# google/guetzli

Hardware: AMD Instinct MI355X
Metric: MPix/s encoded at --quality 95 (higher is better)
Workload: dtype f32+f64 (butteraugli), int32/int16 (DCT/quantize/entropy coding); 1 GPU; single 3840x2160 sRGB image, --quality 95 (BASELINE configs[2]), whole guetzli::Process per step (host RGB in, JPEG bytes out), 1 image per GPU per step; 12 timed steps after 5 warm-up between barrier + synchronise, max over ranks; images_per_gpu=1, steps=12, warmup=5, output_bytes=2895866

## Files before the change

guetzli_amd/csrc/api/chain.h:

```cpp
#pragma once

namespace {
static bool packed_blur(const gz_ctx* c) {
  if (c->cfg.blur_packed >= 0) return c->cfg.blur_packed != 0;
  return (size_t)c->w * c->h >= 1500000;
}
constexpr int kTileRows = 32;
constexpr int kSmallTileRows = 16;
static bool small_tiles(const gz_ctx* c) {
  if (c->cfg.tile_rows == 16) return true;
  if (c->cfg.tile_rows == 32) return false;
  return (size_t)c->w * c->h < 7000000;
}

template <int R, class Src, int NC, bool PAIR = false>
int blur_h(gz_ctx* c, hipStream_t stream, const SrcPack<Src, NC>& src, const PlanePack<NC>& dst,
           const BlurCfg& cfg, const BlurCfg* second = nullptr) {
  if (PAIR != (second != nullptr)) { c->err = "blur pair mismatch"; return GZ_E_STATE; }
  const BlurCfg& cfg1 = PAIR ? *second : cfg;
  if (cfg.r != R || cfg1.r != R) { c->err = "blur radius mismatch"; return GZ_E_STATE; }
  const Taps<R> t0 = taps_of<R>(cfg), t1 = taps_of<R>(cfg1);
  const BorderScale b0 = cfg.bx, b1 = cfg1.bx;
  const int w = c->w, h = c->h, pitch = c->pitch;
  if (packed_blur(c)) {
// ... 77 lines not shown
  make_taps_host(sigma, cfg);
  cfg->border_ratio = border_ratio;
  std::vector<float> xl, xh, yl, yh;
  border_scales_host(*cfg, c->w, &xl, &xh);
  border_scales_host(*cfg, c->h, &yl, &yh);
  const int r = cfg->r;
  if (ctx_owns) TRY(regrow(c, nullptr, nullptr, 0, {{(void**)&cfg->d_scale, sizeof(float) * 4 * r}}));
  else HIPCHK(c, pool_malloc((void**)&cfg->d_scale, sizeof(float) * 4 * r));
  std::vector<float> all;
  all.insert(all.end(), xl.begin(), xl.end());
  all.insert(all.end(), xh.begin(), xh.end());
  all.insert(all.end(), yl.begin(), yl.end());
  all.insert(all.end(), yh.begin(), yh.end());
  HIPCHK(c, hipMemcpy(cfg->d_scale, all.data(), sizeof(float) * 4 * r, hipMemcpyHostToDevice));
  cfg->bx.lo = cfg->d_scale;
  cfg->bx.hi = cfg->d_scale + r;
  cfg->by.lo = cfg->d_scale + 2 * r;
  cfg->by.hi = cfg->d_scale + 3 * r;
  return GZ_OK;
}

static bool single_stream_wanted(const gz_ctx* c) {
  if (c->cfg.single_stream >= 0) return c->cfg.single_stream != 0;
  return slots_taken(c->device) > 1;
}
struct ChainStreams {
  hipStream_t main, side, side2;
};
static ChainStreams chain_streams(const gz_ctx* c, bool forked) {
  return forked ? ChainStreams{c->stream, c->side_stream, c->side_stream2} : ChainStreams{c->stream, c->stream, c->stream};
}
static int record_for(gz_ctx* c, hipStream_t from, hipStream_t to, hipEvent_t ev) {
  if (from != to) HIPCHK(c, hipEventRecord(ev, from));
  return GZ_OK;
}
static int wait_for(gz_ctx* c, hipStream_t from, hipStream_t to, hipEvent_t ev) {
  if (from != to) HIPCHK(c, hipStreamWaitEvent(to, ev, 0));
  return GZ_OK;
}
static int fork(gz_ctx* c, hipStream_t from, hipStream_t to, hipEvent_t ev) {
  TRY(record_for(c, from, to, ev));
  return wait_for(c, from, to, ev);
}

int stage_opsin(gz_ctx* c, hipStream_t stream, const int* tiles = nullptr, int n_tiles = 0) {
  SrcPack<SrcPlain, 3> s;
  for (int i = 0; i < 3; ++i) s.s[i].p = c->lin[i];
  PostOpsin post;
  for (int i = 0; i < 3; ++i) { post.lin[i] = c->lin[i]; post.xyb[i] = c->xyb[i]; }
  return blur2d<2, 3, SrcPlain, PostOpsin>(c, stream, s, post, c->blur[B_OPSIN], BlockMaxOut{nullptr, nullptr, 0, tiles}, n_tiles);
}
static int opsin_tile_rows(const gz_ctx*) { return kSmallTileRows; }

int stage_separate(gz_ctx* c, const ChainStreams& cs, Psycho* ps) {
  c->have_map_plane = false;
  TRY(fork(c, cs.main, cs.side2, c->ev_xyb));
  {
    SrcPack<SrcPlain, 1> s; PlanePack<1> t;
    s.s[0].p = c->xyb[2]; t.p[0] = c->distmap;
    TRY((blur_h<16, SrcPlain, 1>(c, cs.side2, s, t, c->blur[B_LF])));
  }
  {
    SrcPack<SrcPlain, 2> s; PlanePack<2> t; CPlanePack<2> ct;
    for (int i = 0; i < 2; ++i) { s.s[i].p = c->xyb[i]; t.p[i] = c->tmp[i]; ct.p[i] = c->tmp[i]; }
    TRY((blur_h<16, SrcPlain, 2>(c, cs.main, s, t, c->blur[B_LF])));
    PostLFxy post;
    for (int i = 0; i < 2; ++i) { post.lf_raw[i] = c->lf_raw[i]; post.lf_vals[i] = ps->lfv[i]; }
    TRY((blur_v<16, 2, PostLFxy>(c, cs.main, ct, post, c->blur[B_LF])));
  }
  TRY(fork(c, cs.main, cs.side2, c->ev_lfy));
  {
    CPlanePack<1> ct; ct.p[0] = c->distmap;
    PostLFb post; post.lf_raw_y = c->lf_raw[1]; post.lf_vals_b = ps->lfv[2];
    TRY((blur_v<16, 1, PostLFb>(c, cs.side2, ct, post, c->blur[B_LF])));
  }
  {
    SrcPack<SrcDiff, 2> s;
    for (int i = 0; i < 2; ++i) {
      s.s[i].a = c->xyb[i];
      s.s[i].b = c->lf_raw[i];
    }
    PostMF post;
    for (int i = 0; i < 2; ++i) {
      post.xyb[i] = c->xyb[i];
      post.lf_raw[i] = c->lf_raw[i];
      post.mf[i] = ps->mf[i];
      post.hf_pre[i] = c->hfp[i];
    }
    TRY((blur2d<8, 2, SrcDiff, PostMF>(c, cs.main, s, post, c->blur[B_MF])));
  }
  {
    SrcPack<SrcPlain, 2> s;
    for (int i = 0; i < 2; ++i) s.s[i].p = c->hfp[i];
    PostHF post;
    for (int i = 0; i < 2; ++i) {
      post.hf_pre[i] = c->hfp[i];
      post.hf[i] = ps->hf[i];
      post.uhf[i] = ps->uhf[i];
    }
    post.lf_raw_y = c->lf_raw[1];
    TRY((blur2d<4, 2, SrcPlain, PostHF>(c, cs.main, s, post, c->blur[B_HF])));
  }
  return GZ_OK;
}

int stage_mask_blurs(gz_ctx* c, hipStream_t stream, hipStream_t small_stream, const MaskPrePack& pk) {
  dim3 grid(gz_div_up(c->w, 1024), c->h, 2);
  GZ_LAUNCH(k_mask_pre, grid, dim3(256), stream, pk, c->w, c->h, c->pitch);
  KCHK(c);
  TRY(fork(c, stream, small_stream, c->ev_mask_pre));
  {
    SrcPack<SrcPlain, 2> s; PlanePack<2> t; CPlanePack<2> ct;
    s.s[0].p = c->diffx; s.s[1].p = c->diffy;
    t.p[0] = c->tmp[1]; t.p[1] = c->tmp[2];
    ct.p[0] = c->tmp[1]; ct.p[1] = c->tmp[2];
    TRY((blur_h<20, SrcPlain, 2, true>(c, stream, s, t, c->blur[B_MASKX], &c->blur[B_MASKY1])));
    PostStore<2> post; post.out[0] = c->mxb; post.out[1] = c->myb2;
    TRY((blur_v<20, 2, PostStore<2>, true>(c, stream, ct, post, c->blur[B_MASKX], &c->blur[B_MASKY1])));
  }
  {
    SrcPack<SrcPlain, 1> s; s.s[0].p = c->diffy;
// ... 338 lines not shown
```

guetzli_amd/csrc/api/entry_probes.h:

```cpp
#pragma once

extern "C" {

#ifndef GZ_NO_PROBES

int gz_probe_blur(gz_ctx* c, const float* in, float sigma, float border_ratio, float* out) {
  DeviceScope ds_(c);
  if (!c || !in || !out) return GZ_E_ARG;
  BlurCfg cfg;
  int rc = setup_blur_cfg(c, &cfg, sigma, border_ratio, false);
  float* src = c->xyb[0];
  c->xyb_is_cand = false;
  if (rc == GZ_OK) rc = upload_planes(c, in, &src, 1);
  SrcPack<SrcPlain, 1> s; s.s[0].p = src;
  PostStore<1> post; post.out[0] = c->xyb[1];
  if (rc == GZ_OK) rc = blur_plane(c, c->stream, s, c->tmp[0], post, cfg);
  if (rc == GZ_OK) rc = download_plane(c, c->xyb[1], out);
  (void)hipStreamSynchronize(c->stream);
  (void)pool_free(cfg.d_scale);
  return rc;
}

int gz_probe_opsin(gz_ctx* c, const float* rgb3, float* xyb3) {
  DeviceScope ds_(c);
  if (!c || !rgb3 || !xyb3) return GZ_E_ARG;
  c->lin_is_cand = c->xyb_is_cand = false;
  TRY(upload_planes(c, rgb3, c->lin, 3));
  TRY(stage_opsin(c, c->stream));
  for (int i = 0; i < 3; ++i) TRY(download_plane(c, c->xyb[i], xyb3 + (size_t)i * c->w * c->h));
  HIPCHK(c, hipStreamSynchronize(c->stream));
  return GZ_OK;
}

int gz_probe_separate_frequencies(gz_ctx* c, const float* xyb3, float* out10) {
  DeviceScope ds_(c);
  if (!c || !xyb3 || !out10) return GZ_E_ARG;
  TRY(ensure_pip(c));
  c->xyb_is_cand = false;
  TRY(upload_planes(c, xyb3, c->xyb, 3));
  TRY(stage_separate(c, chain_streams(c, false), &c->pip));
  const size_t n = (size_t)c->w * c->h;
  for (int i = 0; i < 3; ++i) TRY(download_plane(c, c->pip.lfv[i], out10 + i * n));
  for (int i = 0; i < 2; ++i) TRY(download_plane(c, c->pip.mf[i], out10 + (3 + i) * n));
  memset(out10 + 5 * n, 0, sizeof(float) * n);
  for (int i = 0; i < 2; ++i) TRY(download_plane(c, c->pip.hf[i], out10 + (6 + i) * n));
  for (int i = 0; i < 2; ++i) TRY(download_plane(c, c->pip.uhf[i], out10 + (8 + i) * n));
  HIPCHK(c, hipStreamSynchronize(c->stream));
  return GZ_OK;
}

int gz_probe_diffmap(gz_ctx* c, const float* rgb0, const float* rgb1, float* diffmap,
                     float* score) {
  DeviceScope ds_(c);
  if (!c || !rgb0 || !rgb1) return GZ_E_ARG;
  TRY(ensure_pip(c));
  c->lin_is_cand = c->xyb_is_cand = false;
  TRY(upload_planes(c, rgb0, c->lin, 3));
  TRY(stage_opsin(c, c->stream));
  TRY(stage_separate(c, chain_streams(c, false), &c->pip));
  TRY(upload_planes(c, rgb1, c->lin, 3));
  TRY(stage_opsin(c, c->stream));
  TRY(stage_separate(c, chain_streams(c, false), &c->pi1));
  TRY(stage_diffmap(c, chain_streams(c, !single_stream_wanted(c)), c->pip, c->pi1, kWantDistmap, ClearMax::kMemset));
  if (diffmap) TRY(download_plane(c, c->distmap, diffmap));
  unsigned bits = 0;
  HIPCHK(c, hipMemcpyAsync(&bits, c->d_max_bits, 4, hipMemcpyDeviceToHost, c->stream));
  HIPCHK(c, hipStreamSynchronize(c->stream));
  if (score) memcpy(score, &bits, 4);
  return GZ_OK;
}

int gz_probe_mask(gz_ctx* c, const float* xyb0, const float* xyb1, float* mask3,
                  float* mask_dc3) {
  DeviceScope ds_(c);
  if (!c || !xyb0 || !xyb1 || !mask3) return GZ_E_ARG;
  TRY(ensure_pip(c));
  float* a[2] = {c->pip.hf[0], c->pip.hf[1]};
  float* b[2] = {c->pi1.hf[0], c->pi1.hf[1]};
  TRY(upload_planes(c, xyb0, a, 2));
  TRY(upload_planes(c, xyb1, b, 2));
  const float* const ca2[2] = {a[0], a[1]};
  const float* const cb2[2] = {b[0], b[1]};
  MaskPrePack pk;
  TRY(mask_pack_plain(c, c->stream, ca2, cb2, &pk));
  TRY(stage_mask_blurs(c, c->stream, c->stream, pk));
  TRY(launch_combine(c, c->stream, combine_mask_args(c, c->mask_out, c->mask_dc_out)));
  const size_t n = (size_t)c->w * c->h;
  for (int i = 0; i < 3; ++i) {
    TRY(download_plane(c, c->mask_out[i], mask3 + i * n));
    if (mask_dc3) TRY(download_plane(c, c->mask_dc_out[i], mask_dc3 + i * n));
  }
  HIPCHK(c, hipStreamSynchronize(c->stream));
  return GZ_OK;
// ... 308 lines not shown
```

guetzli_amd/csrc/gz_kernels_blur.h:

```cpp
#pragma once
#include "gz_common.h"
#include "gz_math.h"

namespace gz {

template <int R>
struct Taps {
  float k[2 * R + 1];
  float ks[2 * R + 1];
};

struct BorderScale {
  const float* lo;
  const float* hi;
};

struct SrcPlain {
  const float* p;
  GZ_DEVFN float operator()(size_t idx) const { return GZ_LDG(p, idx); }
  GZ_DEVFN gz_f4 load4(size_t idx) const { return GZ_LDG4(p, idx); }
};
struct SrcDiff {
  const float* a;
  const float* b;
// ... 490 lines not shown
    if (c > 0) __syncthreads();
    for (int ry = tg; ry < TH + 2 * R; ry += 4) {
      const int y = y0 - R + ry;
      float v = 0.0f;
      if (x < w && y >= 0 && y < h) v = in[(size_t)y * pitch + x];
      tile[ry][tx] = v;
    }
    __syncthreads();
#pragma unroll 1
    for (int i = 0; i < VPTt; ++i) {
      const int ly = tg * VPTt + i;
      const int y = y0 + ly;
      float sum = 0.0f;
      if (y < h) {
        const bool border = y < R || y >= h - R;
        const float* col = &tile[ly][tx];
        if (!border) {
#pragma unroll
          for (int j = 0; j <= 2 * R; ++j) sum += col[j * VW] * taps.ks[j];
        } else {
#pragma unroll
          for (int j = 0; j <= 2 * R; ++j) sum += col[j * VW] * taps.k[j];
          sum = sum * (y < R ? bs.lo[y] : bs.hi[h - 1 - y]);
        }
      }
      if constexpr (ZCH) {
        float* __restrict__ o = bid.z == 1 ? post.out[1] : post.out[0];
        if (x < w && y < h) o[(size_t)y * pitch + x] = sum;
      } else if (NC > 1) {
        outv[c][ly][tx] = sum;
      } else {
        float v1[1] = {sum};
        if (x < w && y < h) (void)post((size_t)y * pitch + x, v1);
      }
    }
  }
  if constexpr (NCL > 1) {
#pragma unroll 1
    for (int i = 0; i < VPTt; ++i) {
      const int ly = tg * VPTt + i;
      const int y = y0 + ly;
      if (x < w && y < h) {
        float v[NC];
#pragma unroll
        for (int c = 0; c < NC; ++c) v[c] = outv[c][ly][tx];
        (void)post((size_t)y * pitch + x, v);
      }
    }
  }
}

constexpr int T2 = 64;

template <int R, int NC, class Src, class Post, bool BM, int TH>
__global__ __launch_bounds__(256, 4) void k_blur2d(SrcPack<Src, NC> src, Post post, int w, int h,
                                                int pitch, Taps<R> taps, BorderScale bsx,
                                                BorderScale bsy, BlockMaxOut bm) {
  constexpr bool ROLL = !BM;
  constexpr int RA = (R + 3) & ~3;
  constexpr int IW = T2 + 2 * RA;
  constexpr int IH = TH + 2 * R;
  constexpr int VPTt = TH / 4;
  constexpr int OFF = RA - R;
  __shared__ __attribute__((aligned(16))) float tile[IH][IW];
  const int tid = threadIdx.x;
  GzTile bid;
  if (bm.tiles) {
    const int t = bm.tiles[blockIdx.x], gx = (w + T2 - 1) / T2;
    bid.x = t % gx; bid.y = t / gx; bid.z = 0;
  } else {
    bid = gz_xcd_tile();
  }
  const int x0 = bid.x * T2, y0 = bid.y * TH;
  const bool interior = x0 >= RA && x0 + T2 + RA <= w && y0 >= R && y0 + TH + R <= h &&
                        (pitch & 3) == 0;
  const int tx = tid & 63, tg = tid >> 6;
  constexpr int kRowSlotShift = (IW / 4) & 15;
  const int hr = tid >> 4;
  const int hq = (((tid & 15) - (hr & 1) * kRowSlotShift) & 15) * 4;
  float acc[ROLL ? 1 : NC][VPTt];
  __shared__ __attribute__((aligned(16))) float outv[ROLL ? NC : 1][ROLL ? TH : 1][T2];
  constexpr int kChannelUnroll = ROLL ? 1 : NC;
#pragma unroll kChannelUnroll
  for (int c = 0; c < NC; ++c) {
    Src s = src.s[0];
#pragma unroll
    for (int k = 1; k < NC; ++k)
      if (c == k) s = src.s[k];
    if (c > 0) __syncthreads();
    if (interior) {
      float kv[2 * R + 1];
#pragma unroll
      for (int j = 0; j <= 2 * R; ++j) kv[j] = GZ_IN_VGPR(taps.ks[j]);
      constexpr int NV = IH * (IW / 4);
      constexpr int SB = 8;
#pragma unroll
      for (int b0 = 0; b0 < NV; b0 += 256 * SB) {
        gz_f4 buf[SB];
#pragma unroll
        for (int k = 0; k < SB; ++k) {
          const int i = b0 + 256 * k + tid;
          if (b0 + 256 * k + 255 < NV || i < NV) {
            const int ry = i / (IW / 4), q = i - ry * (IW / 4);
            buf[k] = s.load4((size_t)(y0 - R + ry) * pitch + (x0 - RA + 4 * q));
          }
        }
#pragma unroll
        for (int k = 0; k < SB; ++k) {
          const int i = b0 + 256 * k + tid;
          if (b0 + 256 * k + 255 < NV || i < NV) {
            const int ry = i / (IW / 4), q = i - ry * (IW / 4);
            *reinterpret_cast<gz_f4*>(&tile[ry][4 * q]) = buf[k];
          }
        }
      }
      __syncthreads();
#pragma unroll 1
      for (int k = 0; k < (IH + 15) / 16; ++k) {
        const int ry = hr + 16 * k;
        const bool on = ry < IH;
        float win[4 + 2 * RA];
        if (on) {
#pragma unroll
          for (int i = 0; i < (4 + 2 * RA) / 4; ++i) {
            const gz_f4 v = *reinterpret_cast<const gz_f4*>(&tile[ry][hq + 4 * i]);
            win[4 * i] = v.v[0]; win[4 * i + 1] = v.v[1]; win[4 * i + 2] = v.v[2]; win[4 * i + 3] = v.v[3];
          }
        }
        GZ_WAVE_LOCKSTEP();
        if (on) {
          gz_f4 o;
#pragma unroll
          for (int i = 0; i < 4; ++i) {
            float sum = 0.0f;
#pragma unroll
            for (int j = 0; j <= 2 * R; ++j) sum += win[OFF + i + j] * kv[j];
            o.v[i] = sum;
          }
          *reinterpret_cast<gz_f4*>(&tile[ry][hq]) = o;
        }
      }
      __syncthreads();
      float win[VPTt + 2 * R];
#pragma unroll
      for (int i = 0; i < VPTt + 2 * R; ++i) win[i] = tile[tg * VPTt + i][tx];
#pragma unroll
      for (int i = 0; i < VPTt; ++i) {
        float sum = 0.0f;
#pragma unroll
        for (int j = 0; j <= 2 * R; ++j) sum += win[i + j] * kv[j];
        if (ROLL) outv[c][tg * VPTt + i][tx] = sum; else acc[c][i] = sum;
      }
    } else {
      for (int i = tid; i < IH * IW; i += 256) {
        const int ry = i / IW, rx = i - ry * IW;
        const int x = x0 - RA + rx, y = y0 - R + ry;
        float v = 0.0f;
        if (x >= 0 && x < w && y >= 0 && y < h) v = s((size_t)y * pitch + x);
        tile[ry][rx] = v;
      }
      __syncthreads();
#pragma unroll 1
      for (int k = 0; k < (IH + 15) / 16; ++k) {
        const int ry = hr + 16 * k;
        const bool on = ry < IH;
        float win[4 + 2 * R];
        if (on) {
#pragma unroll
          for (int i = 0; i < 4 + 2 * R; ++i) win[i] = tile[ry][hq + OFF + i];
        }
        GZ_WAVE_LOCKSTEP();
        if (on) {
#pragma unroll
          for (int i = 0; i < 4; ++i) {
            const int x = x0 + hq + i;
            float sum = 0.0f;
            if (x < w) {
              const bool border = x < R || x >= w - R;
              if (!border) {
#pragma unroll
                for (int j = 0; j <= 2 * R; ++j) sum += win[i + j] * taps.ks[j];
              } else {
#pragma unroll
                for (int j = 0; j <= 2 * R; ++j) sum += win[i + j] * taps.k[j];
                sum = sum * (x < R ? bsx.lo[x] : bsx.hi[w - 1 - x]);
              }
            }
            tile[ry][hq + i] = sum;
          }
        }
      }
      __syncthreads();
      constexpr int kColUnroll = ROLL ? 1 : VPTt;
#pragma unroll kColUnroll
      for (int i = 0; i < VPTt; ++i) {
        const int ly = tg * VPTt + i;
        const int y = y0 + ly;
        float sum = 0.0f;
        if (y < h) {
          const bool border = y < R || y >= h - R;
          const float* col = &tile[ly][tx];
          if (!border) {
#pragma unroll
            for (int j = 0; j <= 2 * R; ++j) sum += col[j * IW] * taps.ks[j];
          } else {
#pragma unroll
            for (int j = 0; j <= 2 * R; ++j) sum += col[j * IW] * taps.k[j];
            sum = sum * (y < R ? bsy.lo[y] : bsy.hi[h - 1 - y]);
          }
        }
        if (ROLL) outv[c][ly][tx] = sum; else acc[c][i] = sum;
      }
    }
  }
  const int x = x0 + tx;
  if (ROLL && !BM) {
    if (x0 + T2 <= w && (pitch & 3) == 0) {
      __syncthreads();
#pragma unroll 1
      for (int q = tid; q < TH * (T2 / 4); q += 256) {
        const int row = q / (T2 / 4), c4 = (q % (T2 / 4)) * 4;
        const int y = y0 + row;
        if (y < h) {
          gz_f4 v[NC];
#pragma unroll
          for (int c = 0; c < NC; ++c) v[c] = *reinterpret_cast<const gz_f4*>(&outv[c][row][c4]);
          post.quad((size_t)y * pitch + x0 + c4, v);
        }
      }
      return;
    }
#pragma unroll 1
    for (int i = 0; i < VPTt; ++i) {
      const int y = y0 + tg * VPTt + i;
      if (x < w && y < h) {
        float v[NC];
#pragma unroll
        for (int c = 0; c < NC; ++c) v[c] = outv[c][tg * VPTt + i][tx];
        (void)post((size_t)y * pitch + x, v);
      }
    }
    return;
  }
  float res[VPTt];
#pragma unroll
  for (int i = 0; i < VPTt; ++i) {
    const int y = y0 + tg * VPTt + i;
    res[i] = 0.0f;
    if (x < w && y < h) {
      float v[NC];
#pragma unroll
      for (int c = 0; c < NC; ++c) v[c] = ROLL ? outv[c][tg * VPTt + i][tx] : acc[c][i];
      res[i] = post((size_t)y * pitch + x, v);
    }
  }
  if constexpr (BM && VPTt == 4) block_max_from_half_columns(res, tx, tg, x0, y0, w, h, bm);
  else if constexpr (BM) block_max_from_registers<VPTt>(res, tx, tg * VPTt, x0, y0, w, h, bm);
}

template <int NC>
struct PostStore {
  float* out[NC];
  GZ_DEVFN float operator()(size_t idx, const float* v) const {
#pragma unroll
    for (int c = 0; c < NC; ++c) out[c][idx] = v[c];
    return v[0];
  }
  GZ_DEVFN void quad(size_t idx, const gz_f4* v) const {
#pragma unroll
    for (int c = 0; c < NC; ++c) GZ_STG4(out[c], idx, v[c]);
  }
  GZ_DEVFN void pair(size_t idx, const float* v0, const float* v1) const {
#pragma unroll
    for (int c = 0; c < NC; ++c) {
      const gz_f2 t = {v0[c], v1[c]};
      GZ_STG2(out[c], idx, t);
    }
  }
};

struct PostOpsin {
  const float* lin[3];
  float* xyb[3];
  GZ_DEVFN float operator()(size_t idx, const float* v) const {
    float x, y, z;
    opsin_pixel(v[0], v[1], v[2], lin[0][idx], lin[1][idx], lin[2][idx], &x, &y, &z);
    xyb[0][idx] = x;
    xyb[1][idx] = y;
    xyb[2][idx] = z;
    return y;
  }
  GZ_DEVFN void pair(size_t idx, const float* v0, const float* v1) const {
    (void)(*this)(idx, v0);
    (void)(*this)(idx + 1, v1);
  }
  GZ_DEVFN void quad(size_t idx, const gz_f4* v) const {
    const gz_f4 l0 = GZ_LDG4(lin[0], idx), l1 = GZ_LDG4(lin[1], idx), l2 = GZ_LDG4(lin[2], idx);
    gz_f4 x, y, z;
#pragma unroll
    for (int i = 0; i < 4; ++i)
      opsin_pixel(v[0].v[i], v[1].v[i], v[2].v[i], l0.v[i], l1.v[i], l2.v[i], &x.v[i], &y.v[i], &z.v[i]);
    GZ_STG4(xyb[0], idx, x);
    GZ_STG4(xyb[1], idx, y);
    GZ_STG4(xyb[2], idx, z);
  }
};

struct PostLFxy {
  float* lf_raw[2];
  float* lf_vals[2];
  GZ_DEVFN float operator()(size_t idx, const float* v) const {
    lf_raw[0][idx] = v[0];
    lf_raw[1][idx] = v[1];
    float vx, vy, vb;
    lf_to_vals(v[0], v[1], 0.0f, &vx, &vy, &vb);
    lf_vals[0][idx] = vx;
    lf_vals[1][idx] = vy;
    return vy;
  }
  GZ_DEVFN void pair(size_t idx, const float* v0, const float* v1) const {
    (void)(*this)(idx, v0);
    (void)(*this)(idx + 1, v1);
  }
  GZ_DEVFN void quad(size_t idx, const gz_f4* v) const {
    GZ_STG4(lf_raw[0], idx, v[0]);
    GZ_STG4(lf_raw[1], idx, v[1]);
    gz_f4 vx, vy;
#pragma unroll
    for (int i = 0; i < 4; ++i) {
      float vb;
      lf_to_vals(v[0].v[i], v[1].v[i], 0.0f, &vx.v[i], &vy.v[i], &vb);
    }
    GZ_STG4(lf_vals[0], idx, vx);
    GZ_STG4(lf_vals[1], idx, vy);
  }
};
struct PostLFb {
  const float* lf_raw_y;
  float* lf_vals_b;
  GZ_DEVFN float operator()(size_t idx, const float* v) const {
    float vx, vy, vb;
    lf_to_vals(0.0f, lf_raw_y[idx], v[0], &vx, &vy, &vb);
    lf_vals_b[idx] = vb;
    return vb;
  }
  GZ_DEVFN void pair(size_t idx, const float* v0, const float* v1) const {
    (void)(*this)(idx, v0);
    (void)(*this)(idx + 1, v1);
  }
  GZ_DEVFN void quad(size_t idx, const gz_f4* v) const {
    const gz_f4 y = GZ_LDG4(lf_raw_y, idx);
    gz_f4 o;
#pragma unroll
    for (int i = 0; i < 4; ++i) {
      float vx, vy;
      lf_to_vals(0.0f, y.v[i], v[0].v[i], &vx, &vy, &o.v[i]);
    }
    GZ_STG4(lf_vals_b, idx, o);
  }
};

struct PostMF {
  const float* xyb[2];
  const float* lf_raw[2];
  float* mf[2];
  float* hf_pre[2];
  GZ_DEVFN float operator()(size_t idx, const float* v) const {
    const float band0 = xyb[0][idx] - lf_raw[0][idx];
    const float band1 = xyb[1][idx] - lf_raw[1][idx];
    const float h0 = band0 - v[0];
    const float h1 = band1 - v[1];
    mf[0][idx] = remove_range((float)0.120079806822, v[0]);
    mf[1][idx] = amplify_range((float)0.03430529365, v[1]);
    hf_pre[0][idx] = suppress_x_by_y(h0, h1);
    hf_pre[1][idx] = h1;
    return h1;
  }
  GZ_DEVFN void pair(size_t idx, const float* v0, const float* v1) const {
    (void)(*this)(idx, v0);
    (void)(*this)(idx + 1, v1);
  }
  GZ_DEVFN void quad(size_t idx, const gz_f4* v) const {
    const gz_f4 x0 = GZ_LDG4(xyb[0], idx), x1 = GZ_LDG4(xyb[1], idx);
    const gz_f4 l0 = GZ_LDG4(lf_raw[0], idx), l1 = GZ_LDG4(lf_raw[1], idx);
    gz_f4 m0, m1, p0, p1;
#pragma unroll
    for (int i = 0; i < 4; ++i) {
// ... 23 lines not shown
    const float kMulRegHf = (float)0.478741530298;
    const float kRegHf = 2000 * kMulRegHf;
    const float kMulSuppressUhf = (float)1.76905001176;
    const float kMulRegUhf = (float)0.310148420674;
    const float kRegUhf = 2000 * kMulRegUhf;
    uhf[0][idx] = hf_pre[0][idx] - v[0];
    hf[0][idx] = remove_range((float)0.0287615200377, v[0]);
    const float br = lf_raw_y[idx];
    float u = hf_pre[1][idx] - v[1];
    float hv = maximum_clamp(v[1], (float)78.8223237675);
    u = maximum_clamp(u, (float)5.8907152736);
    u = suppress_bright(u, br, kMulSuppressUhf, kRegUhf);
    hv = suppress_bright(hv, br, kMulSuppressHf, kRegHf);
    uhf[1][idx] = u;
    hf[1][idx] = hv;
    return hv;
  }
  GZ_DEVFN void pair(size_t idx, const float* v0, const float* v1) const {
    (void)(*this)(idx, v0);
    (void)(*this)(idx + 1, v1);
  }
  GZ_DEVFN void quad(size_t idx, const gz_f4* v) const {
    const float kMulSuppressHf = (float)1.10684769012;
    const float kMulRegHf = (float)0.478741530298;
    const float kRegHf = 2000 * kMulRegHf;
    const float kMulSuppressUhf = (float)1.76905001176;
    const float kMulRegUhf = (float)0.310148420674;
    const float kRegUhf = 2000 * kMulRegUhf;
    const gz_f4 p0 = GZ_LDG4(hf_pre[0], idx), p1 = GZ_LDG4(hf_pre[1], idx), br4 = GZ_LDG4(lf_raw_y, idx);
    gz_f4 u0, h0, u1, h1;
#pragma unroll
    for (int i = 0; i < 4; ++i) {
      u0.v[i] = p0.v[i] - v[0].v[i];
      h0.v[i] = remove_range((float)0.0287615200377, v[0].v[i]);
      const float br = br4.v[i];
      float u = p1.v[i] - v[1].v[i];
      float hv = maximum_clamp(v[1].v[i], (float)78.8223237675);
      u = maximum_clamp(u, (float)5.8907152736);
      u = suppress_bright(u, br, kMulSuppressUhf, kRegUhf);
      hv = suppress_bright(hv, br, kMulSuppressHf, kRegHf);
      u1.v[i] = u;
      h1.v[i] = hv;
    }
    GZ_STG4(uhf[0], idx, u0);
    GZ_STG4(hf[0], idx, h0);
    GZ_STG4(uhf[1], idx, u1);
    GZ_STG4(hf[1], idx, h1);
  }
};

struct PostDiffmapMix {
  const float* d;
  float* out;
  GZ_DEVFN float operator()(size_t idx, const float* v) const {
    const double mul1 = 0.458794906198;
    const float scale = (float)(1.0f / (1.0f + mul1));
    float r = d[idx];
    r = (float)((double)r + mul1 * (double)v[0]);
    r = r * scale;
    if (out) out[idx] = r;
    return r;
  }
  GZ_DEVFN void pair(size_t idx, const float* v0, const float* v1) const {
    (void)(*this)(idx, v0);
    (void)(*this)(idx + 1, v1);
  }
  GZ_DEVFN void quad(size_t idx, const gz_f4* v) const {
    for (int i = 0; i < 4; ++i) { float one[1] = {v[0].v[i]}; (void)(*this)(idx + i, one); }
  }
};


}
```

guetzli_amd/csrc/gz_kernels_search.h:

```cpp
#pragma once
#include "gz_common.h"
#include "gz_kernels_block.h"
#include "gz_kernels_blur.h"
#include "gz_math.h"

namespace gz {

GZ_CONST double kCsf8x8[37] = {
  0.0, 0.0, 0.0, 0.0,
  0.3831134973, 0.676303603859, 1.1550451483, 8,
  8, 0.692062533689, 0.847511538605, 0.498250875965, 0.36198671102, 0.308982169883,
  0.1312701920435, 4.71274312228,
  1.1550451483, 0.847511538605, 4.71274312228, 0.991205724152, 1.30229591239,
  0.627264168628, 0.4, 0.1312701920435,
  0.676303603859, 0.498250875965, 0.991205724152, 0.5, 0.3831134973, 0.349686450518,
  0.627264168628, 0.308982169883,
  0.3831134973, 0.36198671102, 1.30229591239, 0.3831134973, 0.323078800177,
};

struct Cpx {
  double re, im;
};

#define GZ_SQRT_HALF 0.70710678118654752440084436210484903
// ... 27 lines not shown
  const double R2 = a[6].re + a[2].re, dR26 = a[2].re - a[6].re;
  const double a6im = dI04 - dR26, a4im = dI04 + dR26;
  const double dI26 = a[2].im - a[6].im, I2 = a[6].im + a[2].im;
  const double dR04 = a[0].re - a[4].re, R0 = a[4].re + a[0].re;
  const double a4re = dR04 - dI26, a6re = dR04 + dI26;
  const double dR15 = a[1].re - a[5].re, R1 = a[5].re + a[1].re;
  const double dI37 = a[3].im - a[7].im, I3 = a[7].im + a[3].im;
  const double u1 = dR15 - dI37, u3 = dR15 + dI37;
  const double dI15 = a[1].im - a[5].im, I1 = a[5].im + a[1].im;
  const double dR37 = a[3].re - a[7].re, R3 = a[7].re + a[3].re;
  const double u2 = dI15 - dR37, u4 = dI15 + dR37;
  const double m6 = (u1 - u4) * GZ_SQRT_HALF;
  const double m1 = (u1 + u4) * GZ_SQRT_HALF;
  const double m5 = (u2 - u3) * GZ_SQRT_HALF;
  const double m2 = (u2 + u3) * GZ_SQRT_HALF;
  const double e = R2 + R0, o = R3 + R1, t1 = R0 - R2, t3 = R1 - R3;
  const double f = I2 + I0, g = I3 + I1, t2 = I0 - I2, t4 = I1 - I3;
  F[0].re = e + o;       F[0].im = f + g;
  F[1].re = m2 + a6re;   F[1].im = m5 + a6im;
  F[2].re = t1 + t4;     F[2].im = t2 - t3;
  F[3].re = a4re - m6;   F[3].im = a4im - m1;
  F[4].re = e - o;       F[4].im = f - g;
  F[5].re = a6re - m2;   F[5].im = a6im - m5;
  F[6].re = t1 - t4;     F[6].im = t2 + t3;
  F[7].re = m6 + a4re;   F[7].im = m1 + a4im;
}

struct SearchArgs {
  const int16_t* coeffs;
  const int32_t* rank_cnt;
  const uint8_t* rank_idx;
  const uint8_t* rgb;
  const float* srgb_lut;
  const float* block_mask;
  int w, h, bw, nb;
  int coff[3];
  int cbw;
  const uint8_t* samples;
  int lookahead;
  float limit;
  Taps<2> taps;
  float scale_lo[2], scale_hi[2];
  int32_t* out_cnt;
  uint8_t* out_idx;
  float* out_err;
};

constexpr int kEvalBatch = 3;

struct SearchLds {
  short coef[192];
  alignas(16) short coefT[192];
  alignas(16) short col16[64];
  unsigned char ycc[4][64];
  unsigned char list[192];
  unsigned char oidx[192];
  float oerr[192];
  int cpx[64];
  float tmp[3][96];
  double d[kEvalBatch][3][64];
  double red[kEvalBatch][3];
  float err[kEvalBatch];
  int num;
};
static_assert(sizeof(SearchLds) <= 160 * 1024 / 16, "k_block_search: four wavefronts per SIMD need <= 10 KB each");

template <bool ON>
struct SearchLds420 {
  int s10[2][ON ? 100 : 1];
  short cellsrc[ON ? 100 : 2];
};

template <class T>
GZ_DEVFN void idct_component(SearchLds& s, int c, int zero_k, int lane, T* dst) {
  const int iy = lane >> 3, ix = lane & 7;
  const gz_u4 m_row = gz_load_u4(&kIdctMP[4 * iy]), m_col = gz_load_u4(&kIdctMP[4 * ix]);
  const int zt = ((zero_k & 7) << 3) | ((zero_k >> 3) & 7);
  if (lane == 0 && zero_k >= 0) s.coefT[64 * c + zt] = 0;
  __syncthreads();
  const gz_u4 q = gz_load_u4(&s.coefT[64 * c + 8 * ix]);
  s.col16[lane] = (short)((idct_dot8(m_row, q) + (1 << 10)) >> 11);
  __syncthreads();
  if (lane == 0 && zero_k >= 0) s.coefT[64 * c + zt] = s.coef[64 * c + zero_k];
  const gz_u4 r = gz_load_u4(&s.col16[8 * iy]);
  dst[lane] = (T)clamp255((idct_dot8(m_col, r) + (257 << 17)) >> 18);
  __syncthreads();
}

struct Blur8 {
  float wx[5], wy[5], sx, sy;
};
GZ_DEVFN void blur8_axis(int pos, const SearchArgs& a, float* w, float* scale) {
  const bool interior = pos >= 2 && pos < 6;
#pragma unroll
  for (int j = 0; j < 5; ++j) {
    const int p = pos - 2 + j;
    w[j] = interior ? a.taps.ks[j] : (p >= 0 && p < 8 ? a.taps.k[j] : 0.0f);
  }
  const float lo = pos == 0 ? a.scale_lo[0] : a.scale_lo[1];
  const float hi = pos == 7 ? a.scale_hi[0] : a.scale_hi[1];
  *scale = interior ? 1.0f : (pos < 2 ? lo : hi);
}
GZ_DEVFN Blur8 blur8_init(SearchLds& s, int lane, const SearchArgs& a) {
  Blur8 w;
  blur8_axis(lane & 7, a, w.wx, &w.sx);
  blur8_axis(lane >> 3, a, w.wy, &w.sy);
#pragma unroll
// ... 48 lines not shown
}
GZ_DEVFN int upsampled_pixel(const int* s10, int lx, int ly) {
  const int col = (lx >> 1) + 1, row = (ly >> 1) + 1;
  const int dx = (lx & 1) ? 1 : -1, dy = (ly & 1) ? 10 : -10;
  const int i = row * 10 + col;
  const int p = s10[i] * 9 + s10[i + dy] * 3 + s10[i + dx] * 3 + s10[i + dx + dy];
  return (p + 8 - (lx & 1)) >> 4;
}

struct SearchLane {
  Blur8 w;
  double x0[3];
};
GZ_DEVFN SearchLane search_lane_init(SearchLds& s, int lane, int xmin, int ymin, const SearchArgs& a) {
  SearchLane L;
  L.w = blur8_init(s, lane, a);
  const int iy = lane >> 3, ix = lane & 7;
  const int x = xmin + ix < a.w - 1 ? xmin + ix : a.w - 1;
  const int y = ymin + iy < a.h - 1 ? ymin + iy : a.h - 1;
  const uint8_t* p = a.rgb + ((size_t)y * a.w + x) * 3;
  __syncthreads();
  float x0, y0, z0;
  opsin8x8(s, lane, L.w, GZ_LDG(a.srgb_lut, p[0]), GZ_LDG(a.srgb_lut, p[1]), GZ_LDG(a.srgb_lut, p[2]),
           &x0, &y0, &z0);
  L.x0[0] = (double)x0;
  L.x0[1] = (double)y0;
  L.x0[2] = (double)z0;
  return L;
}

struct SearchView {
  int vw, vh;
  int off_x, off_y;
  float m0, m1, m2;
  bool in_image;
};

template <int MODE>
GZ_DEVFN void eval_wide(SearchLds& s, SearchLds420<MODE == 2>& q, int ci, int slot, int lane,
                        const SearchView& v, const SearchLane& L, const int* ring, const SearchArgs& a) {
  const int cc = ci >= 192 ? 0 : ci >> 6, kk = ci >= 192 ? -1 : ci & 63;
  const int iy = lane >> 3, ix = lane & 7;
  const int sx = ix < v.vw ? ix : v.vw - 1, sy = iy < v.vh ? iy : v.vh - 1;
  const int sp = 8 * sy + sx;
  int py, pcb, pcr;
  if constexpr (MODE == 2) {
    idct_component(s, cc, kk, lane, s.cpx);
    fill_s10(q, cc, s.cpx, ring + 100 * (cc - 1), lane);
    const int px = upsampled_pixel(q.s10[cc - 1], 8 * v.off_x + sx, 8 * v.off_y + sy);
    py = s.ycc[0][sp];
    pcb = (cc == 1 ? px : s.ycc[1][sp]) - 128;
    pcr = (cc == 2 ? px : s.ycc[2][sp]) - 128;
  } else {
    idct_component(s, cc, kk, lane, s.ycc[3]);
    const unsigned char* px = &s.ycc[0][0];
    py = px[(cc == 0 ? 192 : 0) + sp];
    pcb = (int)px[(cc == 1 ? 192 : 64) + sp] - 128;
    pcr = (int)px[(cc == 2 ? 192 : 128) + sp] - 128;
  }
  const int half = 1 << 15;
  const int r = clamp255(py + ((GZ_MUL24(91881, pcr) + half) >> 16));
  const int g = clamp255(py + ((GZ_MUL24(-46802, pcr) + (GZ_MUL24(-22554, pcb) + half)) >> 16));
  const int b = clamp255(py + ((GZ_MUL24(116130, pcb) + half) >> 16));
  float x, y, z;
  opsin8x8(s, lane, L.w, GZ_LDG(a.srgb_lut, r), GZ_LDG(a.srgb_lut, g), GZ_LDG(a.srgb_lut, b), &x, &y, &z);
  s.d[slot][0][lane] = L.x0[0] - (double)x;
  s.d[slot][1][lane] = L.x0[1] - (double)y;
  s.d[slot][2][lane] = L.x0[2] - (double)z;
  __syncthreads();
}

GZ_DEVFN void eval_narrow(SearchLds& s, int nc, int lane, const SearchView& v) {
  const int slot9 = lane / 3, ch9 = lane - 3 * slot9;
  double dc_term = 0.0;
  if (lane < 3 * nc) {
    const double* p = s.d[slot9][ch9];
    double sum = 0.0;
    for (int i = 0; i < 64; ++i) sum += p[i];
    const double avg = sum / 64;
    dc_term = (4.0 * avg) * avg;
  }
  __syncthreads();
  for (int t = lane; t < 24 * nc; t += 64) {
    double* p = &s.d[t / 24][(t % 24) >> 3][8 * (t & 7)];
    Cpx F[8];
    real_fft8(p[0], p[1], p[2], p[3], p[4], p[5], p[6], p[7], F);
    p[0] = F[0].re; p[1] = F[4].re;
    p[2] = F[1].re; p[3] = F[1].im;
    p[4] = F[2].re; p[5] = F[2].im;
    p[6] = F[3].re; p[7] = F[3].im;
  }
  __syncthreads();
  double pw8[8];
  if (lane < 15 * nc) {
    const int sl = lane / 15, r = lane - 15 * sl;
    const int ch = r / 5, k = r - 5 * ch;
    const double* col = s.d[sl][ch];
    Cpx F[8];
    if (k == 0 || k == 4) {
      const int j = k == 0 ? 0 : 1;
      real_fft8(col[j], col[8 + j], col[16 + j], col[24 + j], col[32 + j], col[40 + j],
                col[48 + j], col[56 + j], F);
    } else {
      Cpx in[8];
#pragma unroll
      for (int x2 = 0; x2 < 8; ++x2) {
        in[x2].re = col[8 * x2 + 2 * k];
        in[x2].im = col[8 * x2 + 2 * k + 1];
      }
      fft8(in, F);
    }
#pragma unroll
    for (int x2 = 0; x2 < 8; ++x2) {
      const double pv = F[x2].re * F[x2].re + F[x2].im * F[x2].im;
      pw8[x2] = pv * 0.000064;
    }
  }
  __syncthreads();
  if (lane < 15 * nc) {
    const int sl = lane / 15, r = lane - 15 * sl;
    const int ch = r / 5, k = r - 5 * ch;
#pragma unroll
    for (int x2 = 0; x2 < 8; ++x2) s.d[sl][ch][8 * k + x2] = pw8[x2];
  }
  __syncthreads();
  if (lane < 3 * nc) {
    const double* pw = s.d[slot9][ch9];
    double acc = dc_term;
    for (int i = 4; i < 37; ++i) acc += kCsf8x8[i] * pw[i];
    s.red[slot9][ch9] = acc;
  }
  __syncthreads();
  if (lane < nc) {
    double diff = 0.0;
    diff += s.red[lane][0] * (double)v.m0;
    diff += s.red[lane][1] * (double)v.m1;
    diff += s.red[lane][2] * (double)v.m2;
    s.err[lane] = (float)sqrt(diff);
  }
  __syncthreads();
}

template <int MODE>
__global__ __launch_bounds__(MODE == 2 ? 256 : 64, 4) void k_block_search(SearchArgs a) {
  constexpr int NW = MODE == 2 ? 4 : 1;
  __shared__ SearchLds sh[NW];
  __shared__ SearchLds420<MODE == 2> sq[NW];
  __shared__ int s_ring[MODE == 2 ? 200 : 1];
  __shared__ float s_err[kEvalBatch][4];
  const int wave = MODE == 2 ? (int)(threadIdx.x >> 6) : 0, lane = threadIdx.x & 63;
  SearchLds& s = sh[wave];
  SearchLds420<MODE == 2>& q = sq[wave];
  const int blk = blockIdx.x;
  const int gw = MODE == 2 ? a.cbw : a.bw;
  const int gbx = blk % gw, gby = blk / gw;
  SearchView v;
  v.off_x = wave & 1;
  v.off_y = wave >> 1;
  const int bx = MODE == 2 ? 2 * gbx + v.off_x : gbx, by = MODE == 2 ? 2 * gby + v.off_y : gby;
  const int xmin = 8 * bx, ymin = 8 * by;
  v.in_image = xmin < a.w && ymin < a.h;
  v.vw = a.w - xmin < 8 ? a.w - xmin : 8;
  v.vh = a.h - ymin < 8 ? a.h - ymin : 8;
  if (v.vw < 1) v.vw = 1;
// ... 60 lines not shown
  while (n > 0) {
    float best_err = 1e17f;
    int best_i = 0;
    const int tries = n < a.lookahead ? n : a.lookahead;
    for (int base = 0; base < tries; base += kEvalBatch) {
      const int nc = tries - base < kEvalBatch ? tries - base : kEvalBatch;
      for (int j = 0; j < nc; ++j) eval_wide<MODE>(s, q, (int)s.list[base + j], j, lane, v, L, s_ring, a);
      eval_narrow(s, nc, lane, v);
      if (MODE == 2) {
        if (lane < nc) s_err[lane][wave] = v.in_image ? s.err[lane] : 0.0f;
        __syncthreads();
      }
      for (int j = 0; j < nc; ++j) {
        float max_err = 0.0f;
        if (MODE == 2) {
          for (int k = 0; k < 4; ++k) max_err = s_err[j][k] > max_err ? s_err[j][k] : max_err;
        } else {
          const float e = s.err[j];
          max_err = e > 0.0f ? e : 0.0f;
        }
        if (max_err < best_err) {
          best_err = max_err;
          best_i = base + j;
        }
      }
      if (MODE == 2) __syncthreads();
    }
    const int ci = (int)s.list[best_i];
    __syncthreads();
    if (lane == 0) {
      s.coef[ci] = 0;
      s.coefT[(ci & 192) + ((ci & 7) << 3) + ((ci >> 3) & 7)] = 0;
      s.oidx[m] = (unsigned char)ci;
      s.oerr[m] = best_err;
    }
    for (int base = 0; base < n; base += 64) {
      const int j = base + lane;
      unsigned char vv = 0;
      const bool mv = j >= best_i && j < n - 1;
      if (mv) vv = s.list[j + 1];
      __syncthreads();
      if (mv) s.list[j] = vv;
      __syncthreads();
    }
    ++m;
    --n;
    if constexpr (MODE == 2) {
      const int c = ci >> 6;
      idct_component(s, c, -1, lane, s.cpx);
      fill_s10(q, c, s.cpx, s_ring + 100 * (c - 1), lane);
      s.ycc[c][lane] = (unsigned char)upsampled_pixel(q.s10[c - 1], 8 * v.off_x + ix, 8 * v.off_y + iy);
      __syncthreads();
    } else {
      idct_component(s, ci >> 6, -1, lane, s.ycc[ci >> 6]);
    }
  }
  __syncthreads();
  if (lane == 0) {
    float min_err = 1e10f;
    for (int i = m - 1; i >= 0; --i) {
      min_err = s.oerr[i] < min_err ? s.oerr[i] : min_err;
      s.oerr[i] = min_err;
    }
    int num = 0;
    while (num < m && s.oerr[num] <= a.limit) ++num;
    s.num = num;
    if (wave == 0) a.out_cnt[blk] = num;
  }
  __syncthreads();
  const int num = wave == 0 ? s.num : 0;
  for (int i = lane; i < num; i += 64) {
    a.out_idx[(size_t)blk * 192 + i] = s.oidx[i];
    a.out_err[(size_t)blk * 192 + i] = s.oerr[i];
  }
}

__global__ __launch_bounds__(64) void k_compare_blocks(SearchArgs a, const int32_t* __restrict__ block_xy,
                                                       const int16_t* __restrict__ blocks, int n,
                                                       double* __restrict__ out) {
  __shared__ SearchLds s;
  const int i = blockIdx.x, lane = threadIdx.x;
  const int bx = block_xy[2 * i], by = block_xy[2 * i + 1];
  const int xmin = 8 * bx, ymin = 8 * by;
  for (int c = 0; c < 3; ++c) {
    const short cv = blocks[((size_t)i * 3 + c) * 64 + lane];
    s.coef[64 * c + lane] = cv;
    s.coefT[64 * c + 8 * (lane & 7) + (lane >> 3)] = cv;
  }
  __syncthreads();
  const SearchLane L = search_lane_init(s, lane, xmin, ymin, a);
  for (int c = 1; c < 3; ++c) idct_component(s, c, -1, lane, s.ycc[c]);
  SearchView v;
  v.off_x = v.off_y = 0;
  v.in_image = true;
  v.vw = a.w - xmin < 8 ? a.w - xmin : 8;
  v.vh = a.h - ymin < 8 ? a.h - ymin : 8;
  const int mb = by * a.bw + bx;
  v.m0 = a.block_mask[mb];
  v.m1 = a.block_mask[a.nb + mb];
  v.m2 = a.block_mask[2 * a.nb + mb];
  SearchLds420<false> q;
  eval_wide<0>(s, q, 192, 0, lane, v, L, nullptr, a);
  eval_narrow(s, 1, lane, v);
  if (lane == 0) {
    double diff = 0.0;
    diff += s.red[0][0] * (double)v.m0;
    diff += s.red[0][1] * (double)v.m1;
// ... 87 lines not shown
```

Measured before the change: 34.40 MPix/s.

## Skip unused LF-Y stores, reuse centre samples, per-slot candidate pixels in search

```diff
diff --git a/guetzli_amd/csrc/api/chain.h b/guetzli_amd/csrc/api/chain.h
--- a/guetzli_amd/csrc/api/chain.h
+++ b/guetzli_amd/csrc/api/chain.h
@@ -153,7 +153,7 @@
 }
 static int opsin_tile_rows(const gz_ctx*) { return kSmallTileRows; }
 
-int stage_separate(gz_ctx* c, const ChainStreams& cs, Psycho* ps) {
+int stage_separate(gz_ctx* c, const ChainStreams& cs, Psycho* ps, bool lf_y_vals = false) {
   c->have_map_plane = false;
   TRY(fork(c, cs.main, cs.side2, c->ev_xyb));
   {
@@ -165,9 +165,20 @@
     SrcPack<SrcPlain, 2> s; PlanePack<2> t; CPlanePack<2> ct;
     for (int i = 0; i < 2; ++i) { s.s[i].p = c->xyb[i]; t.p[i] = c->tmp[i]; ct.p[i] = c->tmp[i]; }
     TRY((blur_h<16, SrcPlain, 2>(c, cs.main, s, t, c->blur[B_LF])));
-    PostLFxy post;
+    PostLFxy<false> post;
     for (int i = 0; i < 2; ++i) { post.lf_raw[i] = c->lf_raw[i]; post.lf_vals[i] = ps->lfv[i]; }
-    TRY((blur_v<16, 2, PostLFxy>(c, cs.main, ct, post, c->blur[B_LF])));
+    if (lf_y_vals) {
+#ifndef GZ_NO_PROBES
+      PostLFxy<true> all;
+      for (int i = 0; i < 2; ++i) { all.lf_raw[i] = post.lf_raw[i]; all.lf_vals[i] = post.lf_vals[i]; }
+      TRY((blur_v<16, 2, PostLFxy<true>>(c, cs.main, ct, all, c->blur[B_LF])));
+#else
+      c->err = "LF-Y vals: a build without probes";
+      return GZ_E_STATE;
+#endif
+    } else {
+      TRY((blur_v<16, 2, PostLFxy<false>>(c, cs.main, ct, post, c->blur[B_LF])));
+    }
   }
   TRY(fork(c, cs.main, cs.side2, c->ev_lfy));
   {
diff --git a/guetzli_amd/csrc/api/entry_probes.h b/guetzli_amd/csrc/api/entry_probes.h
--- a/guetzli_amd/csrc/api/entry_probes.h
+++ b/guetzli_amd/csrc/api/entry_probes.h
@@ -38,7 +38,7 @@
   TRY(ensure_pip(c));
   c->xyb_is_cand = false;
   TRY(upload_planes(c, xyb3, c->xyb, 3));
-  TRY(stage_separate(c, chain_streams(c, false), &c->pip));
+  TRY(stage_separate(c, chain_streams(c, false), &c->pip, true));
   const size_t n = (size_t)c->w * c->h;
   for (int i = 0; i < 3; ++i) TRY(download_plane(c, c->pip.lfv[i], out10 + i * n));
   for (int i = 0; i < 2; ++i) TRY(download_plane(c, c->pip.mf[i], out10 + (3 + i) * n));
diff --git a/guetzli_amd/csrc/gz_kernels_blur.h b/guetzli_amd/csrc/gz_kernels_blur.h
--- a/guetzli_amd/csrc/gz_kernels_blur.h
+++ b/guetzli_amd/csrc/gz_kernels_blur.h
@@ -566,6 +566,12 @@
 
 constexpr int T2 = 64;
 
+template <class Post>
+struct PostTakesCentre { static constexpr bool value = false; };
+struct PostDiffmapMix;
+template <>
+struct PostTakesCentre<PostDiffmapMix> { static constexpr bool value = true; };
+
 template <int R, int NC, class Src, class Post, bool BM, int TH>
 __global__ __launch_bounds__(256, 4) void k_blur2d(SrcPack<Src, NC> src, Post post, int w, int h,
                                                 int pitch, Taps<R> taps, BorderScale bsx,
@@ -593,6 +599,9 @@
   const int hr = tid >> 4;
   const int hq = (((tid & 15) - (hr & 1) * kRowSlotShift) & 15) * 4;
   float acc[ROLL ? 1 : NC][VPTt];
+  constexpr bool CENTRE = PostTakesCentre<Post>::value;
+  static_assert(!CENTRE || (NC == 1 && !ROLL), "centre samples: one plane, results in registers");
+  float ctr[CENTRE ? VPTt : 1];
   __shared__ __attribute__((aligned(16))) float outv[ROLL ? NC : 1][ROLL ? TH : 1][T2];
   constexpr int kChannelUnroll = ROLL ? 1 : NC;
 #pragma unroll kChannelUnroll
@@ -629,6 +638,11 @@
         }
       }
       __syncthreads();
+      if constexpr (CENTRE) {
+#pragma unroll
+        for (int i = 0; i < VPTt; ++i) ctr[i] = tile[R + tg * VPTt + i][RA + tx];
+        __syncthreads();
+      }
 #pragma unroll 1
       for (int k = 0; k < (IH + 15) / 16; ++k) {
         const int ry = hr + 16 * k;
@@ -674,6 +688,11 @@
         tile[ry][rx] = v;
       }
       __syncthreads();
+      if constexpr (CENTRE) {
+#pragma unroll
+        for (int i = 0; i < VPTt; ++i) ctr[i] = tile[R + tg * VPTt + i][RA + tx];
+        __syncthreads();
+      }
 #pragma unroll 1
       for (int k = 0; k < (IH + 15) / 16; ++k) {
         const int ry = hr + 16 * k;
@@ -765,7 +784,8 @@
       float v[NC];
 #pragma unroll
       for (int c = 0; c < NC; ++c) v[c] = ROLL ? outv[c][tg * VPTt + i][tx] : acc[c][i];
-      res[i] = post((size_t)y * pitch + x, v);
+      if constexpr (CENTRE) res[i] = post((size_t)y * pitch + x, v, ctr[i]);
+      else res[i] = post((size_t)y * pitch + x, v);
     }
   }
   if constexpr (BM && VPTt == 4) block_max_from_half_columns(res, tx, tg, x0, y0, w, h, bm);
@@ -820,6 +840,7 @@
   }
 };
 
+template <bool YVALS>
 struct PostLFxy {
   float* lf_raw[2];
   float* lf_vals[2];
@@ -829,7 +850,7 @@
     float vx, vy, vb;
     lf_to_vals(v[0], v[1], 0.0f, &vx, &vy, &vb);
     lf_vals[0][idx] = vx;
-    lf_vals[1][idx] = vy;
+    if constexpr (YVALS) lf_vals[1][idx] = vy;
     return vy;
   }
   GZ_DEVFN void pair(size_t idx, const float* v0, const float* v1) const {
@@ -846,7 +867,7 @@
       lf_to_vals(v[0].v[i], v[1].v[i], 0.0f, &vx.v[i], &vy.v[i], &vb);
     }
     GZ_STG4(lf_vals[0], idx, vx);
-    GZ_STG4(lf_vals[1], idx, vy);
+    if constexpr (YVALS) GZ_STG4(lf_vals[1], idx, vy);
   }
 };
 struct PostLFb {
@@ -976,15 +997,16 @@
 struct PostDiffmapMix {
   const float* d;
   float* out;
-  GZ_DEVFN float operator()(size_t idx, const float* v) const {
+  GZ_DEVFN float operator()(size_t idx, const float* v, float centre) const {
     const double mul1 = 0.458794906198;
     const float scale = (float)(1.0f / (1.0f + mul1));
-    float r = d[idx];
+    float r = centre;
     r = (float)((double)r + mul1 * (double)v[0]);
     r = r * scale;
     if (out) out[idx] = r;
     return r;
   }
+  GZ_DEVFN float operator()(size_t idx, const float* v) const { return (*this)(idx, v, d[idx]); }
   GZ_DEVFN void pair(size_t idx, const float* v0, const float* v1) const {
     (void)(*this)(idx, v0);
     (void)(*this)(idx + 1, v1);
diff --git a/guetzli_amd/csrc/gz_kernels_search.h b/guetzli_amd/csrc/gz_kernels_search.h
--- a/guetzli_amd/csrc/gz_kernels_search.h
+++ b/guetzli_amd/csrc/gz_kernels_search.h
@@ -103,7 +103,7 @@
   short coef[192];
   alignas(16) short coefT[192];
   alignas(16) short col16[64];
-  unsigned char ycc[4][64];
+  unsigned char ycc[3 + kEvalBatch][64];
   unsigned char list[192];
   unsigned char oidx[192];
   float oerr[192];
@@ -258,11 +258,12 @@
     pcb = (cc == 1 ? px : s.ycc[1][sp]) - 128;
     pcr = (cc == 2 ? px : s.ycc[2][sp]) - 128;
   } else {
-    idct_component(s, cc, kk, lane, s.ycc[3]);
+    idct_component(s, cc, kk, lane, s.ycc[3 + slot]);
     const unsigned char* px = &s.ycc[0][0];
-    py = px[(cc == 0 ? 192 : 0) + sp];
-    pcb = (int)px[(cc == 1 ? 192 : 64) + sp] - 128;
-    pcr = (int)px[(cc == 2 ? 192 : 128) + sp] - 128;
+    const int cand = 192 + 64 * slot;
+    py = px[(cc == 0 ? cand : 0) + sp];
+    pcb = (int)px[(cc == 1 ? cand : 64) + sp] - 128;
+    pcr = (int)px[(cc == 2 ? cand : 128) + sp] - 128;
   }
   const int half = 1 << 15;
   const int r = clamp255(py + ((GZ_MUL24(91881, pcr) + half) >> 16));
@@ -303,19 +304,16 @@
     const int ch = r / 5, k = r - 5 * ch;
     const double* col = s.d[sl][ch];
     Cpx F[8];
-    if (k == 0 || k == 4) {
-      const int j = k == 0 ? 0 : 1;
-      real_fft8(col[j], col[8 + j], col[16 + j], col[24 + j], col[32 + j], col[40 + j],
-                col[48 + j], col[56 + j], F);
-    } else {
-      Cpx in[8];
-#pragma unroll
-      for (int x2 = 0; x2 < 8; ++x2) {
-        in[x2].re = col[8 * x2 + 2 * k];
-        in[x2].im = col[8 * x2 + 2 * k + 1];
-      }
-      fft8(in, F);
-    }
+    const bool real = k == 0 || k == 4;
+    const int jr = real ? k >> 2 : 2 * k, ji = real ? jr : jr + 1;
+    Cpx in[8];
+#pragma unroll
+    for (int x2 = 0; x2 < 8; ++x2) {
+      in[x2].re = col[8 * x2 + jr];
+      const double im = col[8 * x2 + ji];
+      in[x2].im = real ? 0.0 : im;
+    }
+    fft8(in, F);
 #pragma unroll
     for (int x2 = 0; x2 < 8; ++x2) {
       const double pv = F[x2].re * F[x2].re + F[x2].im * F[x2].im;
@@ -482,7 +480,13 @@
       s.ycc[c][lane] = (unsigned char)upsampled_pixel(q.s10[c - 1], 8 * v.off_x + ix, 8 * v.off_y + iy);
       __syncthreads();
     } else {
-      idct_component(s, ci >> 6, -1, lane, s.ycc[ci >> 6]);
+      const int last_base = ((tries - 1) / kEvalBatch) * kEvalBatch;
+      if (best_i >= last_base) {
+        s.ycc[ci >> 6][lane] = s.ycc[3 + best_i - last_base][lane];
+        __syncthreads();
+      } else {
+        idct_component(s, ci >> 6, -1, lane, s.ycc[ci >> 6]);
+      }
     }
   }
   __syncthreads();
```

Measured after the change: 34.94 MPix/s (median of 6 runs). No clear change (+1.6%).
